# arkworks-rs/groth16

Hardware: AMD Instinct MI355X
Metric: R1CS constraints/sec (create_proof, BLS12-381) (higher is better)
Workload: dtype u32-limb Montgomery integers (Fr 255-bit, Fq 381-bit); 1 GPU; SYN(k=22) synthetic R1CS, 4194302 constraints, FFT domain 2^22, bls12_381, full create_proof (7 NTTs + 4 G1 MSMs + 1 G2 MSM), valid proving key generated on the GPU from seeded toxic waste; curve=bls12_381, log2_domain=22, constraints=4194302, key=valid, witness=resident in HBM at entry (--full: value_incl_h2d holds the PCIe-inclusive rates), parallelism=single-gpu

## Files before the change

### groth16_amd/csrc/msm.hip

```cpp
#include "internal.hpp"
#include "msm_common.hpp"
#include "fp30.hpp"
#include "batch_affine.hpp"
#include "window_tables.hpp"
#include <algorithm>
#include <cstdlib>

namespace g16 {

static constexpr int SORT_THREADS = 1024;
static constexpr int ACC_THREADS = 64;
static constexpr int RED_THREADS = 64;
static constexpr int WIN_THREADS = 256;
#ifndef G16_REDUCE_G
#define G16_REDUCE_G 8
#endif
static constexpr uint32_t REDUCE_G = G16_REDUCE_G;

struct PlanDev {
    int c, W;
    uint32_t B;
    uint32_t K[10];
    uint32_t shard_n, shard_r, shard_magic;
};
// ... 81 lines not shown
    __syncthreads();
    const uint64_t i = (uint64_t)blockIdx.x * CLASS_THREADS + threadIdx.x;
    if (i < n) {
        biased_scalar(scalars[i], plan, sw);
        for (int w = 0; w < plan.W; ++w) {
            uint32_t key, neg;
            if (digit_to_bucket(window_of(sw, w, plan.c), plan.c, &key, &neg) && shard_local_key(plan, &key)) atomicAdd(&cnt[key >> blog], 1u);
        }
    }
    __syncthreads();
    if (threadIdx.x < Q) block_counts[(uint64_t)threadIdx.x * gridDim.x + blockIdx.x] = cnt[threadIdx.x];
}

template <class Fr>
__global__ __launch_bounds__(CLASS_THREADS) void class_partition_kernel(const Fr* __restrict__ scalars, uint64_t n, PlanDev plan, uint32_t blog,
                                                                        uint32_t Q, const uint32_t* __restrict__ block_off,
                                                                        uint16_t* __restrict__ ent_key, uint32_t* __restrict__ ent_tag) {
    __shared__ uint32_t sw[MSM_SWORDS][CLASS_THREADS];
    __shared__ uint32_t cur[MAX_CLASSES];
    if (threadIdx.x < Q) cur[threadIdx.x] = block_off[(uint64_t)threadIdx.x * gridDim.x + blockIdx.x];
    __syncthreads();
    const uint64_t i = (uint64_t)blockIdx.x * CLASS_THREADS + threadIdx.x;
    if (i >= n) return;
    biased_scalar(scalars[i], plan, sw);
    for (int w = 0; w < plan.W; ++w) {
        uint32_t key, neg;
        if (digit_to_bucket(window_of(sw, w, plan.c), plan.c, &key, &neg) && shard_local_key(plan, &key)) {
            const uint32_t pos = atomicAdd(&cur[key >> blog], 1u);
            ent_key[pos] = (uint16_t)((key & ((1u << blog) - 1u)) | (neg << 15));
            ent_tag[pos] = (uint32_t)i | ((uint32_t)w << 26);
        }
    }
}

static __global__ __launch_bounds__(SORT_M_THREADS) void bucket_count_merged_kernel(const uint16_t* __restrict__ ent_key,
                                                                           const uint32_t* __restrict__ class_off, uint32_t nb, uint32_t B,
                                                                           uint32_t* __restrict__ wg_counts) {
    extern __shared__ __attribute__((aligned(16))) unsigned char smem[];
    uint32_t* hist = reinterpret_cast<uint32_t*>(smem);
    const uint32_t q = blockIdx.y;
    const uint32_t lo = class_off[(uint64_t)q * nb], hi = class_off[(uint64_t)(q + 1) * nb];
    for (uint32_t b = threadIdx.x; b < B; b += SORT_M_THREADS) hist[b] = 0;
    __syncthreads();
    for (uint64_t p = (uint64_t)lo + blockIdx.x * SORT_M_THREADS + threadIdx.x; p < hi; p += (uint64_t)gridDim.x * SORT_M_THREADS)
        atomicAdd(&hist[ent_key[p] & 0x7fffu], 1u);
    __syncthreads();
    uint32_t* out = wg_counts + ((uint64_t)q * gridDim.x + blockIdx.x) * B;
    for (uint32_t b = threadIdx.x; b < B; b += SORT_M_THREADS) out[b] = hist[b];
}

static __global__ __launch_bounds__(256) void bucket_wg_scan_kernel(uint32_t* __restrict__ wg_counts, uint32_t G, uint32_t B, uint32_t M,
                                                                    uint32_t* __restrict__ counts) {
    const uint32_t i = blockIdx.x * 256 + threadIdx.x;
    if (i >= M) return;
    const uint32_t q = i / B, b = i - q * B;
    uint32_t* col = wg_counts + (uint64_t)q * G * B + b;
    uint32_t run = 0;
    for (uint32_t x = 0; x < G; ++x) {
        const uint32_t v = col[(uint64_t)x * B];
        col[(uint64_t)x * B] = run;
        run += v;
    }
    counts[i] = run;
}

static __global__ __launch_bounds__(SORT_M_THREADS) void bucket_scatter_merged_kernel(const uint16_t* __restrict__ ent_key,
                                                                             const uint32_t* __restrict__ ent_tag,
                                                                             const uint32_t* __restrict__ class_off, uint32_t nb, uint32_t B,
                                                                             const uint32_t* __restrict__ offsets,
                                                                             const uint32_t* __restrict__ wg_counts, uint32_t* __restrict__ sorted) {
    extern __shared__ __attribute__((aligned(16))) unsigned char smem[];
    uint32_t* hist = reinterpret_cast<uint32_t*>(smem);
    const uint32_t q = blockIdx.y;
    const uint32_t lo = class_off[(uint64_t)q * nb], hi = class_off[(uint64_t)(q + 1) * nb];
    if ((uint64_t)lo + (uint64_t)blockIdx.x * SORT_M_THREADS >= hi) return;
    const uint64_t qb = (uint64_t)q * B;
    const uint32_t* mine = wg_counts + ((uint64_t)q * gridDim.x + blockIdx.x) * B;
    for (uint32_t b = threadIdx.x; b < B; b += SORT_M_THREADS) hist[b] = offsets[qb + b] + mine[b];
    __syncthreads();
    const uint64_t first = (uint64_t)lo + blockIdx.x * SORT_M_THREADS + threadIdx.x, step = (uint64_t)gridDim.x * SORT_M_THREADS;
    for (uint64_t p = first; p < hi; p += step) {
        const uint32_t d = ent_key[p];
        const uint32_t pos = atomicAdd(&hist[d & 0x7fffu], 1u);
        sorted[pos] = ent_tag[p] | ((d >> 15) << 31);
    }
}

static constexpr int SCAN_THREADS = 256;
static constexpr int SCAN_PER_THREAD = 8;
static constexpr int SCAN_TILE = SCAN_THREADS * SCAN_PER_THREAD;
static constexpr uint32_t HEAVY_PARTS = 16;

__device__ __forceinline__ uint32_t block_exclusive(uint32_t v, uint32_t* sh, uint32_t* total) {
    const uint32_t tid = threadIdx.x;
    sh[tid] = v;
    __syncthreads();
    for (uint32_t d = 1; d < SCAN_THREADS; d <<= 1) {
        const uint32_t add = tid >= d ? sh[tid - d] : 0u;
        __syncthreads();
        sh[tid] += add;
        __syncthreads();
    }
    const uint32_t incl = sh[tid];
    *total = sh[SCAN_THREADS - 1];
    __syncthreads();
    return incl - v;
}

static __global__ __launch_bounds__(SCAN_THREADS) void scan_block_sums_kernel(const uint32_t* __restrict__ vals, uint32_t M, uint32_t pad,
                                                                       uint32_t* __restrict__ block_sums) {
    __shared__ uint32_t sa[SCAN_THREADS];
    const uint32_t base = blockIdx.x * SCAN_TILE + threadIdx.x * SCAN_PER_THREAD;
    uint32_t sum = 0, tot;
    G16_UNROLL for (int j = 0; j < SCAN_PER_THREAD; ++j) sum += (base + j < M) ? ((vals[base + j] + pad) & ~pad) : 0u;
    (void)block_exclusive(sum, sa, &tot);
    if (threadIdx.x == 0) block_sums[blockIdx.x] = tot;
}

static __global__ __launch_bounds__(SCAN_THREADS) void scan_block_offsets_kernel(uint32_t* __restrict__ block_sums, uint32_t nblocks, uint32_t M,
                                                                          uint32_t* __restrict__ prefix) {
    __shared__ uint32_t sa[SCAN_THREADS];
    uint32_t carry = 0;
    for (uint32_t base = 0; base < nblocks; base += SCAN_THREADS) {
        const uint32_t i = base + threadIdx.x;
        const uint32_t a = i < nblocks ? block_sums[i] : 0u;
        uint32_t tot;
        const uint32_t ea = block_exclusive(a, sa, &tot);
        if (i < nblocks) block_sums[i] = carry + ea;
        carry += tot;
    }
    if (threadIdx.x == 0) prefix[M] = carry;
}

static __global__ __launch_bounds__(SCAN_THREADS) void scan_write_kernel(const uint32_t* __restrict__ vals, uint32_t M, uint32_t pad,
                                                                  const uint32_t* __restrict__ block_base, uint32_t* __restrict__ prefix) {
    __shared__ uint32_t sa[SCAN_THREADS];
    const uint32_t base = blockIdx.x * SCAN_TILE + threadIdx.x * SCAN_PER_THREAD;
    uint32_t cv[SCAN_PER_THREAD], sum = 0, tot;
    G16_UNROLL for (int j = 0; j < SCAN_PER_THREAD; ++j) { cv[j] = (base + j < M) ? ((vals[base + j] + pad) & ~pad) : 0u; sum += cv[j]; }
    uint32_t a = block_base[blockIdx.x] + block_exclusive(sum, sa, &tot);
    G16_UNROLL for (int j = 0; j < SCAN_PER_THREAD; ++j) {
        if (base + j < M) { prefix[base + j] = a; a += cv[j]; }
    }
}

static __global__ void bucket_slots_kernel(const uint32_t* __restrict__ offsets, uint32_t M, uint32_t off_shift, uint32_t lseg,
                                    uint32_t* __restrict__ nparts, uint32_t* __restrict__ heavy ) {
    const uint32_t b = blockIdx.x * blockDim.x + threadIdx.x;
    if (b >= M) return;
    const uint32_t lo = offsets[b] >> off_shift, hi = offsets[b + 1] >> off_shift;
    const uint32_t np = hi > lo ? ((hi - 1) / lseg - lo / lseg + 1u) : 0u;
    nparts[b] = np;
    if (np > HEAVY_PARTS) heavy[1 + atomicAdd(&heavy[0], 1u)] = b;
}

static __global__ __launch_bounds__(SORT_THREADS) void bucket_scatter_kernel(const uint16_t* __restrict__ planes, uint64_t n, uint32_t chunk,
                                                                      int c, uint32_t B, const uint32_t* __restrict__ offsets,
                                                                      uint32_t* __restrict__ cursor, uint32_t* __restrict__ sorted) {
    extern __shared__ __attribute__((aligned(16))) unsigned char smem[];
    uint32_t* hist = reinterpret_cast<uint32_t*>(smem);
    const int w = blockIdx.y;
    for (uint32_t b = threadIdx.x; b < B; b += SORT_THREADS) hist[b] = 0;
    __syncthreads();
    const uint64_t lo = (uint64_t)blockIdx.x * chunk, hi = min(n, lo + chunk);
    const uint16_t* plane = planes + (uint64_t)w * n;
    for (uint64_t p = lo + threadIdx.x; p < hi; p += SORT_THREADS) {
        uint32_t bucket, neg;
        if (digit_to_bucket(plane[p], c, &bucket, &neg)) atomicAdd(&hist[bucket], 1u);
    }
    __syncthreads();
    const uint64_t wb = (uint64_t)w * B;
    for (uint32_t b = threadIdx.x; b < B; b += SORT_THREADS) {
        const uint32_t v = hist[b];
        if (v) hist[b] = offsets[wb + b] + atomicAdd(&cursor[wb + b], v);
    }
    __syncthreads();
    for (uint64_t p = lo + threadIdx.x; p < hi; p += SORT_THREADS) {
        uint32_t bucket, neg;
        if (digit_to_bucket(plane[p], c, &bucket, &neg)) {
            const uint32_t pos = atomicAdd(&hist[bucket], 1u);
            sorted[pos] = (uint32_t)p | (neg << 31);
        }
    }
}

template <class F30>
struct LdsAccStore {
    static constexpr int NL = F30::PREFIX_LIMBS;
    static constexpr int QUADS = NL / 4, TAIL = NL % 4;
    static constexpr int WORDS_PER_VALUE = NL * ACC_THREADS;
    uint32_t* quad;
    uint32_t* tail;
    __device__ __forceinline__ F30 ld(int v) const {
        asm volatile("" ::: "memory");
        uint32_t w[NL];
        const uint32_t* q = quad + v * WORDS_PER_VALUE;
        G16_UNROLL for (int g = 0; g < QUADS; ++g) {
            const uint4 t = *reinterpret_cast<const uint4*>(q + g * 4 * ACC_THREADS);
            w[4 * g] = t.x; w[4 * g + 1] = t.y; w[4 * g + 2] = t.z; w[4 * g + 3] = t.w;
        }
        const uint32_t* r = tail + v * WORDS_PER_VALUE;
        G16_UNROLL for (int i = 0; i < TAIL; ++i) w[4 * QUADS + i] = r[i * ACC_THREADS];
        return F30::from_limbs(w);
    }
    __device__ __forceinline__ void st(int v, const F30& a) const {
        uint32_t w[NL];
        a.get_limbs(w);
        uint32_t* q = quad + v * WORDS_PER_VALUE;
        G16_UNROLL for (int g = 0; g < QUADS; ++g)
            *reinterpret_cast<uint4*>(q + g * 4 * ACC_THREADS) = make_uint4(w[4 * g], w[4 * g + 1], w[4 * g + 2], w[4 * g + 3]);
        uint32_t* r = tail + v * WORDS_PER_VALUE;
        G16_UNROLL for (int i = 0; i < TAIL; ++i) r[i * ACC_THREADS] = w[4 * QUADS + i];
        asm volatile("" ::: "memory");
    }
};

template <class F30>
struct RawAccStore {
    AccRaw<typename F30::Raw>* p;
    __device__ __forceinline__ F30 ld(int k) const {
        asm volatile("" ::: "memory");
        if constexpr (F30::LANES_PER_TASK == 1) {
            static_assert(sizeof(F30) == sizeof(typename F30::Raw), "one-lane fields share the raw layout");
            return reinterpret_cast<const F30*>(p)[k];
        } else {
            typedef typename F30::B B30;
            return F30{reinterpret_cast<const B30*>(p)[2 * k + (F30::lane_hi() ? 1 : 0)]};
        }
    }
    __device__ __forceinline__ void st(int k, const F30& a) const {
        if constexpr (F30::LANES_PER_TASK == 1) {
            reinterpret_cast<F30*>(p)[k] = a;
        } else {
            typedef typename F30::B B30;
            reinterpret_cast<B30*>(p)[2 * k + (F30::lane_hi() ? 1 : 0)] = a.c;
        }
        asm volatile("" ::: "memory");
    }
    __device__ __forceinline__ bool inf() const {
        const F30 zz = ld(2);
        if constexpr (F30::LANES_PER_TASK == 1) return zz.raw_zero();
        else return F30::both(zz.c.raw_zero());
    }
    __device__ __forceinline__ void set_inf() const { st(2, F30::zero()); }
};
template <class F30>
struct RegAccStore {
    F30 v[4];
    __device__ __forceinline__ F30 ld(int k) const { return v[k]; }
    __device__ __forceinline__ void st(int k, const F30& a) { v[k] = a; }
};
template <class F30, class St>
__device__ __forceinline__ Acc30<F30> gather_acc(const St& st, bool inf) {
    Acc30<F30> a;
    a.inf = inf;
    if (inf) { a.x = a.y = a.zz = a.zzz = F30::zero(); return a; }
    a.x = st.ld(0); a.y = st.ld(1); a.zz = st.ld(2); a.zzz = st.ld(3);
    return a;
}

static constexpr int PASS_BATCH = 4;
template <class F30>
struct PassBatch {
    const Affine<typename F30::Std>* bases[PASS_BATCH];
    int64_t shift[PASS_BATCH];
    uint64_t base_count[PASS_BATCH];
    const uint32_t* sorted[PASS_BATCH];
    const uint32_t* offsets[PASS_BATCH];
    const uint32_t* slot_off[PASS_BATCH];
    AccRaw<typename F30::Raw>* partials[PASS_BATCH];
};

template <class F30, bool DIRECT>
__global__ __launch_bounds__(ACC_THREADS, F30::ACC_MIN_WAVES) void bucket_accumulate30_kernel(
    PassBatch<F30> batch, uint32_t M, uint32_t off_shift, uint32_t lseg, uint32_t merged) {
    const Affine<typename F30::Std>* __restrict__ bases = batch.bases[blockIdx.y];
    const int64_t shift = batch.shift[blockIdx.y];
    const uint64_t base_count = batch.base_count[blockIdx.y];
    const uint32_t* __restrict__ sorted = batch.sorted[blockIdx.y];
    const uint32_t* __restrict__ offsets = batch.offsets[blockIdx.y];
    const uint32_t* __restrict__ slot_off = batch.slot_off[blockIdx.y];
    AccRaw<typename F30::Raw>* __restrict__ partials = batch.partials[blockIdx.y];
    const uint32_t t = (blockIdx.x * ACC_THREADS + threadIdx.x) / F30::LANES_PER_TASK;
    const uint32_t S = offsets[M] >> off_shift;
    const uint64_t start64 = (uint64_t)t * lseg;
    if (start64 >= S) return;
    const uint32_t start = (uint32_t)start64;
    const uint32_t end = (uint32_t)min((uint64_t)S, start64 + lseg);
    uint32_t lo = 0, hi = M;
    while (hi - lo > 1) {
        const uint32_t mid = (lo + hi) >> 1;
        if ((offsets[mid] >> off_shift) <= start) lo = mid; else hi = mid;
    }
    uint32_t b = lo, b_first = offsets[b] >> off_shift, b_end = offsets[b + 1] >> off_shift;
    __shared__ __attribute__((aligned(16))) uint32_t acc_lds[4 * F30::PREFIX_LIMBS * ACC_THREADS];
    AccParked<F30, LdsAccStore<F30>> acc;
    acc.s.quad = acc_lds + 4 * threadIdx.x;
    acc.s.tail = acc_lds + 4 * LdsAccStore<F30>::QUADS * ACC_THREADS + threadIdx.x;
    acc.inf = true;
    auto flush = [&](AccRaw<typename F30::Raw>* dst) { acc.gather().store_raw(dst); acc.inf = true; };
    uint32_t v_next = 0;
    typedef typename F30::PackedC YNext;
    F30 px_next = F30::zero();
    YNext py_next = YNext::zero();
    bool ok_next = false;
    auto decode = [&](uint32_t v, int64_t* at) -> bool {
// ... 266 lines not shown
}

int make_msm_plan(uint64_t n, int scalar_bits, const uint32_t* modulus_words, int mod_nwords, int merged_c, MsmPlan* plan, int shard_n,
                  int shard_r) {
    if (shard_n < 1 || shard_n > 64 || shard_r < 0 || shard_r >= shard_n || (shard_n > 1 && merged_c <= 0)) return G16_ERR_INTERNAL;
    int c = merged_c;
    if (c <= 0) {
        c = msm_window_override();
        if (c <= 0) {
            double best = 1e300;
            for (int cc = 4; cc <= 16; ++cc) {
                const int W = plan_windows(cc, scalar_bits, modulus_words, mod_nwords, nullptr);
                if (W < 0) continue;
                const double t = plan_cost(n, W, (double)W * (1u << (cc - 1)), W);
                if (t < best) { best = t; c = cc; }
            }
        }
        if (c < 3) c = 3;
        if (c > 16) c = 16;
    } else if (c < MSM_MERGED_MIN_C || c > MSM_MERGED_MAX_C || n > MSM_MERGED_MAX_N) {
        return G16_ERR_INTERNAL;
    }
    const int W = plan_windows(c, scalar_bits, modulus_words, mod_nwords, plan->K);
    if (W < 0 || (merged_c > 0 && W > 32)) return G16_ERR_INTERNAL;
    plan->c = c;
    plan->W = W;
    plan->merged = merged_c > 0;
    plan->shard_n = shard_n;
    plan->shard_r = shard_r;
    if (plan->merged) {
        const uint32_t all = 1u << (c - 1), local = (all + (uint32_t)shard_n - 1) / (uint32_t)shard_n;
        uint32_t B = 1;
        while (B < local && B < (1u << 15)) B <<= 1;
        plan->B = B;
        plan->groups = (int)((local + B - 1) / B);
    } else {
        plan->B = 1u << (c - 1);
        plan->groups = W;
    }
    plan->G = REDUCE_G;
    if (const char* e = getenv("G16_MSM_REDUCE_G")) {
        const int v = atoi(e);
        if (v == 4 || v == 8 || v == 16 || v == 32) plan->G = (uint32_t)v;
    }
    const uint64_t all_entries = n * (uint64_t)W / (uint64_t)shard_n;
    plan->affine_levels = 0;
    {
        const uint64_t mean_load = all_entries / plan->buckets();
        (void)mean_load;
        int R = 0;
        if (const char* e = getenv("G16_MSM_AFFINE_LEVELS")) {
            const int v = atoi(e);
            if (v >= 0 && v <= 4) R = v;
        }
        if (all_entries + (uint64_t)plan->buckets() * ((1u << R) - 1u) >= ((uint64_t)1 << 32)) R = 0;
        if (shard_n > 1) R = 0;
        plan->affine_levels = R;
    }
    const uint64_t entries = (all_entries >> plan->affine_levels) + (plan->affine_levels ? plan->buckets() : 0);
    uint32_t l = 64;
    while (l > 16 && entries / l < 4ull * 131072ull) l >>= 1;
    const uint64_t mean = entries / plan->buckets() + 1;
    while (l < 128 && (uint64_t)l * 4 < mean) l <<= 1;
    if (const char* e = getenv("G16_MSM_SEGMENT")) {
        const int v = atoi(e);
        if (v >= 8 && v <= 4096) l = (uint32_t)v;
    }
    plan->Lmax = l;
    uint64_t nchunks = 2048 / (uint64_t)plan->groups;
    if (nchunks < 1) nchunks = 1;
    uint64_t chunk = (n + nchunks - 1) / nchunks;
    chunk = (chunk + 1023) / 1024 * 1024;
    if (chunk < 1024) chunk = 1024;
    plan->chunk = (uint32_t)chunk;
    return G16_OK;
}

#endif

static int ilog2(uint32_t v) { int l = 0; while ((1u << l) < v) ++l; return l; }

template <class C>
int sort_scalars(const typename C::Fr* d_scalars, uint64_t n, int merged_c, Arena& arena, hipStream_t st, ScalarSort* out, int shard_n,
                 int shard_r) {
    typedef typename C::Fr Fr;
    if (n >= ((uint64_t)1 << 31)) return G16_ERR_BAD_LENGTH;
    uint32_t modw[Fr::N];
    for (int i = 0; i < Fr::N; ++i) modw[i] = Fr::Params::mod(i);
    MsmPlan plan;
    G16_TRY(make_msm_plan(n, Fr::Params::BITS, modw, Fr::N, merged_c, &plan, shard_n, shard_r));
    out->plan = plan;
    out->n = n;
    const uint32_t M = plan.buckets();
    const uint64_t nw = n * (uint64_t)plan.W;
    if (nw >= ((uint64_t)1 << 32)) return G16_ERR_BAD_LENGTH;
    uint16_t* planes = nullptr;
    uint32_t* ent_tag = nullptr;
    uint32_t *class_cnt = nullptr, *class_off = nullptr;
    uint32_t *counts = nullptr, *cursor = nullptr, *nparts = nullptr, *block_sums = nullptr;
    uint32_t sort_class_log = SORT_CLASS_LOG;
    if (const char* e = getenv("G16_SORT_CLASS_LOG")) {
        const int v = atoi(e);
        if (v >= 8 && v <= 15) sort_class_log = (uint32_t)v;
    }
    const uint32_t slog = plan.merged ? std::min<uint32_t>(sort_class_log, (uint32_t)ilog2(plan.B)) : 0u;
    const uint32_t Bs = plan.merged ? 1u << slog : plan.B;
    const uint32_t nb = (uint32_t)((n + CLASS_THREADS - 1) / CLASS_THREADS), Q = plan.merged ? M >> slog : (uint32_t)plan.groups;
    G16_TRY(arena.alloc_n(nw ? nw : 1, &planes));
    if (plan.merged) {
        if (Q > MAX_CLASSES) return G16_ERR_INTERNAL;
        G16_TRY(arena.alloc_n(nw ? nw : 1, &ent_tag));
        G16_TRY(arena.alloc_n((size_t)Q * nb + 1, &class_cnt));
        G16_TRY(arena.alloc_n((size_t)Q * nb + 1, &class_off));
    }
    G16_TRY(arena.alloc_n((size_t)3 * M + 1, &counts));
    cursor = counts + M;
    out->heavy = counts + 2 * (size_t)M;
    G16_TRY(arena.alloc_n((size_t)M + 1, &out->offsets));
    G16_TRY(arena.alloc_n((size_t)M + 1, &out->task_off));
    G16_TRY(arena.alloc_n((size_t)M, &nparts));
    const int R = plan.affine_levels;
    const uint32_t pad = (1u << R) - 1u;
    const uint64_t max_sorted = nw + (uint64_t)M * pad;
    if (max_sorted >= ((uint64_t)1 << 32)) return G16_ERR_BAD_LENGTH;
    out->max_sorted = max_sorted;
    G16_TRY(arena.alloc_n(max_sorted ? max_sorted : 1, &out->sorted));
    if (R) G16_HIP_TRY(hipMemsetAsync(out->sorted, 0xff, max_sorted * sizeof(uint32_t), st));
    const uint64_t walked = R ? (max_sorted >> R) : nw;
    out->max_segments = (uint32_t)((walked + plan.Lmax - 1) / plan.Lmax);
    out->max_tasks = out->max_segments + M;
    G16_HIP_TRY(hipMemsetAsync(counts, 0, ((size_t)2 * M + 1) * sizeof(uint32_t), st));
    PlanDev pd;
    pd.c = plan.c; pd.W = plan.W; pd.B = plan.B;
    for (int k = 0; k < 10; ++k) pd.K[k] = plan.K[k];
    pd.shard_n = (uint32_t)plan.shard_n;
    pd.shard_r = (uint32_t)plan.shard_r;
    pd.shard_magic = plan.shard_n > 1 ? (uint32_t)((((uint64_t)1 << 32) + (uint64_t)plan.shard_n - 1) / (uint64_t)plan.shard_n) : 0u;
    const size_t lds = (size_t)Bs * sizeof(uint32_t);
    static PerDeviceOnce attr_once;
    std::atomic<bool>& attr_set = attr_once.flag();
    if (!attr_set) {
        G16_HIP_TRY(hipFuncSetAttribute(reinterpret_cast<const void*>(&bucket_count_kernel), hipFuncAttributeMaxDynamicSharedMemorySize,
                                        128 * 1024));
        G16_HIP_TRY(hipFuncSetAttribute(reinterpret_cast<const void*>(&bucket_scatter_kernel), hipFuncAttributeMaxDynamicSharedMemorySize,
                                        128 * 1024));
        G16_HIP_TRY(hipFuncSetAttribute(reinterpret_cast<const void*>(&bucket_count_merged_kernel),
                                        hipFuncAttributeMaxDynamicSharedMemorySize, 128 * 1024));
        G16_HIP_TRY(hipFuncSetAttribute(reinterpret_cast<const void*>(&bucket_scatter_merged_kernel),
                                        hipFuncAttributeMaxDynamicSharedMemorySize, 128 * 1024));
        attr_set = true;
    }
    const unsigned nchunks = (unsigned)((n + plan.chunk - 1) / plan.chunk);
    const uint32_t blog = plan.merged ? slog : (uint32_t)ilog2(plan.B);
    const uint32_t max_scan = std::max(M, plan.merged ? Q * nb : 0u);
    G16_TRY(arena.alloc_n((size_t)(max_scan + SCAN_TILE - 1) / SCAN_TILE, &block_sums));
    auto prefix_scan = [&](const uint32_t* vals, uint32_t* prefix, uint32_t count, uint32_t padmask = 0) -> int {
        const uint32_t nblocks = (count + SCAN_TILE - 1) / SCAN_TILE;
        hipLaunchKernelGGL(scan_block_sums_kernel, dim3(nblocks), dim3(SCAN_THREADS), 0, st, vals, count, padmask, block_sums);
        G16_LAUNCH_CHECK();
        hipLaunchKernelGGL(scan_block_offsets_kernel, dim3(1), dim3(SCAN_THREADS), 0, st, block_sums, nblocks, count, prefix);
        G16_LAUNCH_CHECK();
        hipLaunchKernelGGL(scan_write_kernel, dim3(nblocks), dim3(SCAN_THREADS), 0, st, vals, count, padmask, block_sums, prefix);
        G16_LAUNCH_CHECK();
        return G16_OK;
    };
    unsigned gx = std::max(1u, std::min(std::min(4096u / Q, 256u), (unsigned)((nw + SORT_M_THREADS - 1) / SORT_M_THREADS)));
    if (const char* e = getenv("G16_SORT_GX")) {
        const int v = atoi(e);
        if (v >= 1 && v <= 4096) gx = (unsigned)v;
    }
    uint32_t* wg_counts = nullptr;
    if (plan.merged) G16_TRY(arena.alloc_n((size_t)Q * gx * Bs, &wg_counts));
    if (n) {
        if (plan.merged) {
            hipLaunchKernelGGL((class_count_kernel<Fr>), dim3(nb), dim3(CLASS_THREADS), 0, st, d_scalars, n, pd, blog, Q, class_cnt);
            G16_LAUNCH_CHECK();
            G16_TRY(prefix_scan(class_cnt, class_off, Q * nb));
            hipLaunchKernelGGL((class_partition_kernel<Fr>), dim3(nb), dim3(CLASS_THREADS), 0, st, d_scalars, n, pd, blog, Q, class_off, planes,
                               ent_tag);
            G16_LAUNCH_CHECK();
            hipLaunchKernelGGL(bucket_count_merged_kernel, dim3(gx, Q), dim3(SORT_M_THREADS), lds, st, planes, class_off, nb, Bs, wg_counts);
            G16_LAUNCH_CHECK();
            hipLaunchKernelGGL(bucket_wg_scan_kernel, dim3((M + 255) / 256), dim3(256), 0, st, wg_counts, gx, Bs, M, counts);
        } else {
            hipLaunchKernelGGL((digits_kernel<Fr>), dim3((unsigned)((n + 255) / 256)), dim3(256), 0, st, d_scalars, n, pd, planes);
            G16_LAUNCH_CHECK();
            hipLaunchKernelGGL(bucket_count_kernel, dim3(nchunks, plan.W), dim3(SORT_THREADS), lds, st, planes, n, plan.chunk, plan.c, plan.B,
                               counts);
        }
        G16_LAUNCH_CHECK();
    }
    G16_TRY(prefix_scan(counts, out->offsets, M, pad));
    hipLaunchKernelGGL(bucket_slots_kernel, dim3((M + 255) / 256), dim3(256), 0, st, out->offsets, M, (uint32_t)R, plan.Lmax, nparts,
                       out->heavy);
    G16_LAUNCH_CHECK();
    G16_TRY(prefix_scan(nparts, out->task_off, M));
    if (n) {
        if (plan.merged)
            hipLaunchKernelGGL(bucket_scatter_merged_kernel, dim3(gx, Q), dim3(SORT_M_THREADS), lds, st, planes, ent_tag, class_off, nb, Bs,
                               out->offsets, wg_counts, out->sorted);
        else
            hipLaunchKernelGGL(bucket_scatter_kernel, dim3(nchunks, plan.W), dim3(SORT_THREADS), lds, st, planes, n, plan.chunk, plan.c, plan.B,
                               out->offsets, cursor, out->sorted);
        G16_LAUNCH_CHECK();
    }
    return G16_OK;
}

template <class F>
static int alloc_msm_buffers(const ScalarSort& ss, Arena& arena, MsmBuffers<F>* out) {
    typedef AccRaw<typename Lazy30<F>::type::Raw> Raw;
    const MsmPlan& plan = ss.plan;
    const uint32_t cpw = plan.B / plan.chunk_buckets();
    Raw *partials = nullptr, *chunk_out = nullptr;
    G16_TRY(arena.alloc_n((size_t)ss.max_tasks ? ss.max_tasks : 1, &partials));
    G16_TRY(arena.alloc_n((size_t)cpw * plan.groups * 2, &chunk_out));
    G16_TRY(arena.alloc_n((size_t)plan.outputs(), &out->window_sums));
    out->partials = partials;
    out->chunk_out = chunk_out;
    return G16_OK;
}

template <class F>
int msm_bucket_pass(const Affine<F>* d_bases, int64_t shift, uint64_t base_count, const ScalarSort& ss, Arena& arena, hipStream_t st,
                    MsmBuffers<F>* out, EventTimer* bucket_timer) {
    typedef typename Lazy30<F>::type F30;
    typedef AccRaw<typename Lazy30<F>::type::Raw> Raw;
    const MsmPlan& plan = ss.plan;
    const uint32_t M = plan.buckets();
    const int R = plan.affine_levels;
    if (!R || !ss.max_sorted) {
        const PassJob<F> job{d_bases, shift, base_count, &ss, out};
        return msm_bucket_pass_batch<F>(&job, 1, arena, st, bucket_timer);
    }
    G16_TRY(alloc_msm_buffers<F>(ss, arena, out));
    Raw* partials = static_cast<Raw*>(out->partials);
    Affine<F>* lists[2] = {nullptr, nullptr};
    Word4* prefix = nullptr;
    constexpr uint32_t T = 64 / F30::LANES_PER_TASK;
    constexpr int QUADS = AffineLevel<F30, true>::QUADS;
    auto level_K = [&](int r) -> uint32_t {
        const uint64_t pairs = ss.max_sorted >> (r + 1);
        uint32_t K = 64;
        while (K > 8 && pairs / ((uint64_t)K * T) < 2048) K >>= 1;
        return K;
    };
    auto level_waves = [&](int r) -> uint64_t { return ((ss.max_sorted >> (r + 1)) + (uint64_t)level_K(r) * T - 1) / ((uint64_t)level_K(r) * T); };
    {
        G16_TRY(arena.alloc_n((size_t)(ss.max_sorted >> 1) + 1, &lists[0]));
        if (R > 1) G16_TRY(arena.alloc_n((size_t)(ss.max_sorted >> 2) + 1, &lists[1]));
        size_t recs = 0;
        for (int r = 0; r < R; ++r) recs = std::max(recs, (size_t)(level_waves(r) * level_K(r)) * QUADS * 64);
        G16_TRY(arena.alloc_n(recs ? recs : 1, &prefix));
    }
    if (bucket_timer) G16_TRY(bucket_timer->start(st));
    {
        AffineLevelArgs<F30> a;
        a.sorted = ss.sorted;
        a.total = ss.offsets + M;
        a.prefix = prefix;
        a.shift = shift;
        a.base_count = base_count;
        a.merged = plan.merged ? 1u : 0u;
        for (int r = 0; r < R; ++r) {
            a.in = r == 0 ? d_bases : lists[(r - 1) & 1];
            a.out = lists[r & 1];
            a.level = (uint32_t)r;
            a.K = level_K(r);
            const uint64_t waves = level_waves(r);
            const unsigned blocks = (unsigned)((waves * 64 + AFF_THREADS - 1) / AFF_THREADS);
            if (r == 0) hipLaunchKernelGGL((affine_level_kernel<F30, true>), dim3(blocks), dim3(AFF_THREADS), 0, st, a);
            else hipLaunchKernelGGL((affine_level_kernel<F30, false>), dim3(blocks), dim3(AFF_THREADS), 0, st, a);
            G16_LAUNCH_CHECK();
        }
    }
    if (ss.max_segments) {
        const uint64_t lanes = (uint64_t)ss.max_segments * F30::LANES_PER_TASK;
        const dim3 grid((unsigned)((lanes + ACC_THREADS - 1) / ACC_THREADS));
        PassBatch<F30> b;
        for (int i = 0; i < PASS_BATCH; ++i) {
            b.bases[i] = lists[(R - 1) & 1]; b.shift[i] = 0; b.base_count[i] = 0; b.sorted[i] = nullptr;
            b.offsets[i] = ss.offsets; b.slot_off[i] = ss.task_off; b.partials[i] = partials;
        }
        hipLaunchKernelGGL((bucket_accumulate30_kernel<F30, true>), grid, dim3(ACC_THREADS), 0, st, b, M, (uint32_t)R, plan.Lmax, 0u);
        G16_LAUNCH_CHECK();
    }
    if (bucket_timer) G16_TRY(bucket_timer->stop(st));
    return G16_OK;
}

template <class F30>
static unsigned pass_lds_pad() {
    static const int want = [] { const char* e = getenv("G16_PASS_WG_PER_CU"); return e ? atoi(e) : 0; }();
    if (want <= 0) return 0;
    const unsigned own = 4u * F30::PREFIX_LIMBS * ACC_THREADS * 4u;
    const unsigned per = (160u * 1024u / (unsigned)want) & ~255u;
    return per > own ? per - own : 0;
}

template <class F>
int msm_bucket_pass_batch(const PassJob<F>* jobs, int n, Arena& arena, hipStream_t st, EventTimer* bucket_timer) {
    typedef typename Lazy30<F>::type F30;
    typedef AccRaw<typename Lazy30<F>::type::Raw> Raw;
    if (n < 1 || n > PASS_BATCH) return G16_ERR_INTERNAL;
    const MsmPlan& plan = jobs[0].ss->plan;
    for (int i = 0; i < n; ++i) {
        const MsmPlan& q = jobs[i].ss->plan;
        if (q.B != plan.B || q.groups != plan.groups || q.Lmax != plan.Lmax || q.merged != plan.merged) return G16_ERR_INTERNAL;
        if (q.affine_levels && jobs[i].ss->max_sorted) return G16_ERR_INTERNAL;
    }
    PassBatch<F30> b;
    uint32_t max_segments = 0;
    for (int i = 0; i < n; ++i) G16_TRY(alloc_msm_buffers<F>(*jobs[i].ss, arena, jobs[i].out));
    for (int i = 0; i < PASS_BATCH; ++i) {
        const PassJob<F>& j = jobs[i < n ? i : 0];
        b.bases[i] = j.bases; b.shift[i] = j.shift; b.base_count[i] = j.base_count; b.sorted[i] = j.ss->sorted;
        b.offsets[i] = j.ss->offsets; b.slot_off[i] = j.ss->task_off; b.partials[i] = static_cast<Raw*>(j.out->partials);
        if (i < n) max_segments = std::max(max_segments, j.ss->max_segments);
    }
    if (bucket_timer) G16_TRY(bucket_timer->start(st));
    if (max_segments) {
        const uint64_t lanes = (uint64_t)max_segments * F30::LANES_PER_TASK;
        const dim3 grid((unsigned)((lanes + ACC_THREADS - 1) / ACC_THREADS), (unsigned)n);
        hipLaunchKernelGGL((bucket_accumulate30_kernel<F30, false>), grid, dim3(ACC_THREADS), pass_lds_pad<F30>(), st, b, plan.buckets(), 0u,
                           plan.Lmax, plan.merged ? 1u : 0u);
        G16_LAUNCH_CHECK();
    }
    if (bucket_timer) G16_TRY(bucket_timer->stop(st));
    return G16_OK;
}

template <class F>
static int reduce_setup(size_t* lds_heavy, size_t* lds_win) {
    typedef typename Lazy30<F>::type F30;
    typedef AccRaw<typename F30::Raw> Raw;
    static PerDeviceOnce attr_once;
    std::atomic<bool>& attr_set = attr_once.flag();
    *lds_heavy = sizeof(Raw) * HEAVY_THREADS / F30::LANES_PER_TASK;
    *lds_win = sizeof(Raw) * WIN_THREADS / F30::LANES_PER_TASK;
    if (!attr_set) {
        G16_HIP_TRY(hipFuncSetAttribute(reinterpret_cast<const void*>(&heavy_reduce_kernel<F30>), hipFuncAttributeMaxDynamicSharedMemorySize,
                                        (int)*lds_heavy));
        G16_HIP_TRY(hipFuncSetAttribute(reinterpret_cast<const void*>(&window_reduce_kernel<F30>), hipFuncAttributeMaxDynamicSharedMemorySize,
                                        (int)*lds_win));
        attr_set = true;
    }
    return G16_OK;
}

template <class F>
// ... 189 lines not shown
```

Before: 68.09 million constraints/s.

## Replace merged bucket count/scatter with two-level LDS radix sort for MSM buckets

For the merged-plan, unsharded case, the per-workgroup bucket histogram plus global-atomic scatter is replaced by a two-level sort. The first level partitions entries by high key bits into sub-ranges, using per-tile LDS staging so global writes are coalesced. The second level sorts each sub-range in LDS and writes bucket counts and sorted words. This targets scattered global writes and the large wg_counts scan, at the cost of an extra pass over keys and tags, extra buffers, and LDS-capacity assumptions (FINAL_CAP) that fall back to direct global writes when exceeded.

```diff
diff --git a/groth16_amd/csrc/msm.hip b/groth16_amd/csrc/msm.hip
--- a/groth16_amd/csrc/msm.hip
+++ b/groth16_amd/csrc/msm.hip
@@ -257,6 +257,158 @@
     const uint32_t np = hi > lo ? ((hi - 1) / lseg - lo / lseg + 1u) : 0u;
     nparts[b] = np;
     if (np > HEAVY_PARTS) heavy[1 + atomicAdd(&heavy[0], 1u)] = b;
+}
+
+static constexpr uint32_t MAX_SUBS = 256;
+static constexpr uint32_t MAX_SUB_LOG = 7;
+static constexpr uint32_t SUB_TILE = 4096;
+static constexpr uint32_t SUB_PER_LANE = SUB_TILE / SORT_M_THREADS;
+static constexpr uint32_t SUB_BATCH = 4;
+static constexpr uint32_t FINAL_CAP = 10240;
+static constexpr uint32_t FINAL_BATCH = 4;
+static_assert(SORT_M_THREADS == SCAN_THREADS && MAX_SUBS <= SCAN_THREADS && SUB_TILE <= 65536, "block_exclusive scans one value per lane");
+
+__device__ __forceinline__ uint32_t lds_take(uint32_t* ctr, uint32_t idx, bool valid) {
+    const uint64_t act = __ballot(valid);
+    if (act == 0) return 0;
+    const int first = __ffsll((unsigned long long)act) - 1;
+    const uint32_t idx0 = (uint32_t)__shfl((int)idx, first);
+    if (__ballot(valid && idx == idx0) == act) {
+        const uint32_t lane = threadIdx.x & 63u;
+        uint32_t base = 0;
+        if ((int)lane == first) base = atomicAdd(&ctr[idx0], (uint32_t)__popcll(act));
+        base = (uint32_t)__shfl((int)base, first);
+        return base + (uint32_t)__popcll(act & (((uint64_t)1 << lane) - 1u));
+    }
+    return valid ? atomicAdd(&ctr[idx], 1u) : 0u;
+}
+
+static __global__ __launch_bounds__(SORT_M_THREADS) void sub_count_kernel(const uint16_t* __restrict__ ent_key,
+                                                                          const uint32_t* __restrict__ class_off, uint32_t nb, uint32_t S,
+                                                                          uint32_t sublog, uint32_t* __restrict__ sub_counts) {
+    __shared__ uint32_t cnt[MAX_SUBS];
+    const uint32_t q = blockIdx.y;
+    const uint64_t lo = class_off[(uint64_t)q * nb], hi = class_off[(uint64_t)(q + 1) * nb];
+    cnt[threadIdx.x] = 0;
+    __syncthreads();
+    for (uint64_t tlo = lo + (uint64_t)blockIdx.x * SUB_TILE; tlo < hi; tlo += (uint64_t)gridDim.x * SUB_TILE) {
+        uint32_t k[SUB_PER_LANE];
+        G16_UNROLL for (uint32_t j = 0; j < SUB_PER_LANE; ++j) {
+            const uint64_t p = tlo + j * SORT_M_THREADS + threadIdx.x;
+            k[j] = p < hi ? (uint32_t)ent_key[p] : 0xffffffffu;
+        }
+        G16_UNROLL for (uint32_t j = 0; j < SUB_PER_LANE; ++j) (void)lds_take(cnt, (k[j] & 0x7fffu) >> sublog, k[j] != 0xffffffffu);
+    }
+    __syncthreads();
+    if (threadIdx.x < S) sub_counts[((uint64_t)q * S + threadIdx.x) * gridDim.x + blockIdx.x] = cnt[threadIdx.x];
+}
+
+static __global__ __launch_bounds__(SORT_M_THREADS) void sub_partition_kernel(const uint16_t* __restrict__ ent_key,
+                                                                              const uint32_t* __restrict__ ent_tag,
+                                                                              const uint32_t* __restrict__ class_off, uint32_t nb, uint32_t S,
+                                                                              uint32_t sublog, const uint32_t* __restrict__ sub_off,
+                                                                              uint16_t* __restrict__ out_key, uint32_t* __restrict__ out_tag) {
+    __shared__ uint32_t cnt[MAX_SUBS], start[MAX_SUBS], cur[MAX_SUBS], gcur[MAX_SUBS], sa[SCAN_THREADS];
+    __shared__ uint32_t stag[SUB_TILE];
+    __shared__ uint16_t skey[SUB_TILE];
+    const uint32_t q = blockIdx.y;
+    const uint64_t lo = class_off[(uint64_t)q * nb], hi = class_off[(uint64_t)(q + 1) * nb];
+    if (lo + (uint64_t)blockIdx.x * SUB_TILE >= hi) return;
+    gcur[threadIdx.x] = threadIdx.x < S ? sub_off[((uint64_t)q * S + threadIdx.x) * gridDim.x + blockIdx.x] : 0u;
+    cnt[threadIdx.x] = 0;
+    __syncthreads();
+    for (uint64_t tlo = lo + (uint64_t)blockIdx.x * SUB_TILE; tlo < hi; tlo += (uint64_t)gridDim.x * SUB_TILE) {
+        const uint32_t tn = (uint32_t)min((uint64_t)SUB_TILE, hi - tlo);
+        _Pragma("unroll 1") for (uint32_t i0 = 0; i0 < tn; i0 += SUB_BATCH * SORT_M_THREADS) {
+            uint32_t k[SUB_BATCH];
+            G16_UNROLL for (uint32_t j = 0; j < SUB_BATCH; ++j) {
+                const uint32_t i = i0 + j * SORT_M_THREADS + threadIdx.x;
+                k[j] = i < tn ? (uint32_t)ent_key[tlo + i] : 0xffffffffu;
+            }
+            G16_UNROLL for (uint32_t j = 0; j < SUB_BATCH; ++j) (void)lds_take(cnt, (k[j] & 0x7fffu) >> sublog, k[j] != 0xffffffffu);
+        }
+        __syncthreads();
+        uint32_t tot;
+        const uint32_t mine = cnt[threadIdx.x], ex = block_exclusive(mine, sa, &tot);
+        start[threadIdx.x] = ex;
+        cur[threadIdx.x] = ex;
+        __syncthreads();
+        _Pragma("unroll 1") for (uint32_t i0 = 0; i0 < tn; i0 += SUB_BATCH * SORT_M_THREADS) {
+            uint32_t k[SUB_BATCH], t[SUB_BATCH];
+            G16_UNROLL for (uint32_t j = 0; j < SUB_BATCH; ++j) {
+                const uint32_t i = i0 + j * SORT_M_THREADS + threadIdx.x;
+                k[j] = i < tn ? (uint32_t)ent_key[tlo + i] : 0xffffffffu;
+                t[j] = i < tn ? ent_tag[tlo + i] : 0u;
+            }
+            G16_UNROLL for (uint32_t j = 0; j < SUB_BATCH; ++j) {
+                const bool valid = k[j] != 0xffffffffu;
+                const uint32_t pos = lds_take(cur, (k[j] & 0x7fffu) >> sublog, valid);
+                if (valid) {
+                    skey[pos] = (uint16_t)k[j];
+                    stag[pos] = t[j];
+                }
+            }
+        }
+        __syncthreads();
+        _Pragma("unroll 1") for (uint32_t i = threadIdx.x; i < tn; i += SORT_M_THREADS) {
+            const uint32_t key = skey[i], s = (key & 0x7fffu) >> sublog;
+            const uint32_t g = gcur[s] + (i - start[s]);
+            out_key[g] = (uint16_t)key;
+            out_tag[g] = stag[i];
+        }
+        __syncthreads();
+        gcur[threadIdx.x] += mine;
+        cnt[threadIdx.x] = 0;
+        __syncthreads();
+    }
+}
+
+static __global__ __launch_bounds__(SORT_M_THREADS) void final_sort_kernel(const uint16_t* __restrict__ ent_key,
+                                                                           const uint32_t* __restrict__ ent_tag,
+                                                                           const uint32_t* __restrict__ sub_off, uint32_t G, uint32_t sublog,
+                                                                           uint32_t* __restrict__ counts, uint32_t* __restrict__ sorted) {
+    __shared__ uint32_t cnt[1u << MAX_SUB_LOG], cur[1u << MAX_SUB_LOG], sa[SCAN_THREADS];
+    __shared__ uint32_t out[FINAL_CAP];
+    const uint32_t u = blockIdx.x, NB = 1u << sublog;
+    const uint64_t lo = sub_off[(uint64_t)u * G], hi = sub_off[(uint64_t)(u + 1) * G];
+    if (threadIdx.x < NB) cnt[threadIdx.x] = 0;
+    __syncthreads();
+    for (uint64_t base = lo; base < hi; base += 2 * FINAL_BATCH * SORT_M_THREADS) {
+        uint32_t k[2 * FINAL_BATCH];
+        G16_UNROLL for (uint32_t j = 0; j < 2 * FINAL_BATCH; ++j) {
+            const uint64_t p = base + j * SORT_M_THREADS + threadIdx.x;
+            k[j] = p < hi ? (uint32_t)ent_key[p] : 0xffffffffu;
+        }
+        G16_UNROLL for (uint32_t j = 0; j < 2 * FINAL_BATCH; ++j) (void)lds_take(cnt, k[j] & (NB - 1u), k[j] != 0xffffffffu);
+    }
+    __syncthreads();
+    const uint32_t mine = threadIdx.x < NB ? cnt[threadIdx.x] : 0u;
+    if (threadIdx.x < NB) counts[((uint64_t)u << sublog) + threadIdx.x] = mine;
+    uint32_t tot;
+    const uint32_t ex = block_exclusive(mine, sa, &tot);
+    if (threadIdx.x < NB) cur[threadIdx.x] = ex;
+    __syncthreads();
+    const bool resident = hi - lo <= FINAL_CAP;
+    for (uint64_t base = lo; base < hi; base += FINAL_BATCH * SORT_M_THREADS) {
+        uint32_t k[FINAL_BATCH], t[FINAL_BATCH];
+        G16_UNROLL for (uint32_t j = 0; j < FINAL_BATCH; ++j) {
+            const uint64_t p = base + j * SORT_M_THREADS + threadIdx.x;
+            k[j] = p < hi ? (uint32_t)ent_key[p] : 0xffffffffu;
+            t[j] = p < hi ? ent_tag[p] : 0u;
+        }
+        G16_UNROLL for (uint32_t j = 0; j < FINAL_BATCH; ++j) {
+            const bool valid = k[j] != 0xffffffffu;
+            const uint32_t pos = lds_take(cur, k[j] & (NB - 1u), valid), word = t[j] | ((k[j] >> 15) << 31);
+            if (valid) {
+                if (resident) out[pos] = word;
+                else sorted[lo + pos] = word;
+            }
+        }
+    }
+    if (!resident) return;
+    __syncthreads();
+    const uint32_t N = (uint32_t)(hi - lo);
+    for (uint32_t i = threadIdx.x; i < N; i += SORT_M_THREADS) sorted[lo + i] = out[i];
 }
 
 static __global__ __launch_bounds__(SORT_THREADS) void bucket_scatter_kernel(const uint16_t* __restrict__ planes, uint64_t n, uint32_t chunk,
@@ -829,7 +981,20 @@
     }
     const unsigned nchunks = (unsigned)((n + plan.chunk - 1) / plan.chunk);
     const uint32_t blog = plan.merged ? slog : (uint32_t)ilog2(plan.B);
-    const uint32_t max_scan = std::max(M, plan.merged ? Q * nb : 0u);
+    const bool two_level = plan.merged && R == 0;
+    uint32_t sublog = 0, S = 1;
+    unsigned gx2 = 1;
+    if (two_level) {
+        const uint64_t mean_x4 = 4 * (nw / (uint64_t)plan.shard_n) / M + 1;
+        const uint32_t lo_log = slog > 8 ? slog - 8 : 0u;
+        sublog = std::min<uint32_t>(slog, MAX_SUB_LOG);
+        while (sublog > lo_log && (mean_x4 << sublog) > 3 * (uint64_t)FINAL_CAP) --sublog;
+        if (sublog > MAX_SUB_LOG) return G16_ERR_INTERNAL;
+        S = Bs >> sublog;
+        gx2 = std::max(1u, std::min(std::min(4096u / Q, 256u), (unsigned)((nw + SUB_TILE - 1) / SUB_TILE)));
+    }
+    const uint32_t sub_cells = two_level ? Q * S * gx2 : 0u;
+    const uint32_t max_scan = std::max(std::max(M, plan.merged ? Q * nb : 0u), sub_cells);
     G16_TRY(arena.alloc_n((size_t)(max_scan + SCAN_TILE - 1) / SCAN_TILE, &block_sums));
     auto prefix_scan = [&](const uint32_t* vals, uint32_t* prefix, uint32_t count, uint32_t padmask = 0) -> int {
         const uint32_t nblocks = (count + SCAN_TILE - 1) / SCAN_TILE;
@@ -847,7 +1012,15 @@
         if (v >= 1 && v <= 4096) gx = (unsigned)v;
     }
     uint32_t* wg_counts = nullptr;
-    if (plan.merged) G16_TRY(arena.alloc_n((size_t)Q * gx * Bs, &wg_counts));
+    if (plan.merged && !two_level) G16_TRY(arena.alloc_n((size_t)Q * gx * Bs, &wg_counts));
+    uint16_t* sub_key = nullptr;
+    uint32_t *sub_tag = nullptr, *sub_cnt = nullptr, *sub_off = nullptr;
+    if (two_level) {
+        G16_TRY(arena.alloc_n(nw ? nw : 1, &sub_key));
+        G16_TRY(arena.alloc_n(nw ? nw : 1, &sub_tag));
+        G16_TRY(arena.alloc_n((size_t)sub_cells + 1, &sub_cnt));
+        G16_TRY(arena.alloc_n((size_t)sub_cells + 1, &sub_off));
+    }
     if (n) {
         if (plan.merged) {
             hipLaunchKernelGGL((class_count_kernel<Fr>), dim3(nb), dim3(CLASS_THREADS), 0, st, d_scalars, n, pd, blog, Q, class_cnt);
@@ -856,9 +1029,21 @@
             hipLaunchKernelGGL((class_partition_kernel<Fr>), dim3(nb), dim3(CLASS_THREADS), 0, st, d_scalars, n, pd, blog, Q, class_off, planes,
                                ent_tag);
             G16_LAUNCH_CHECK();
-            hipLaunchKernelGGL(bucket_count_merged_kernel, dim3(gx, Q), dim3(SORT_M_THREADS), lds, st, planes, class_off, nb, Bs, wg_counts);
-            G16_LAUNCH_CHECK();
-            hipLaunchKernelGGL(bucket_wg_scan_kernel, dim3((M + 255) / 256), dim3(256), 0, st, wg_counts, gx, Bs, M, counts);
+            if (two_level) {
+                hipLaunchKernelGGL(sub_count_kernel, dim3(gx2, Q), dim3(SORT_M_THREADS), 0, st, planes, class_off, nb, S, sublog, sub_cnt);
+                G16_LAUNCH_CHECK();
+                G16_TRY(prefix_scan(sub_cnt, sub_off, sub_cells));
+                hipLaunchKernelGGL(sub_partition_kernel, dim3(gx2, Q), dim3(SORT_M_THREADS), 0, st, planes, ent_tag, class_off, nb, S, sublog,
+                                   sub_off, sub_key, sub_tag);
+                G16_LAUNCH_CHECK();
+                hipLaunchKernelGGL(final_sort_kernel, dim3(Q * S), dim3(SORT_M_THREADS), 0, st, sub_key, sub_tag, sub_off, gx2, sublog, counts,
+                                   out->sorted);
+            } else {
+                hipLaunchKernelGGL(bucket_count_merged_kernel, dim3(gx, Q), dim3(SORT_M_THREADS), lds, st, planes, class_off, nb, Bs,
+                                   wg_counts);
+                G16_LAUNCH_CHECK();
+                hipLaunchKernelGGL(bucket_wg_scan_kernel, dim3((M + 255) / 256), dim3(256), 0, st, wg_counts, gx, Bs, M, counts);
+            }
         } else {
             hipLaunchKernelGGL((digits_kernel<Fr>), dim3((unsigned)((n + 255) / 256)), dim3(256), 0, st, d_scalars, n, pd, planes);
             G16_LAUNCH_CHECK();
@@ -872,7 +1057,7 @@
                        out->heavy);
     G16_LAUNCH_CHECK();
     G16_TRY(prefix_scan(nparts, out->task_off, M));
-    if (n) {
+    if (n && !two_level) {
         if (plan.merged)
             hipLaunchKernelGGL(bucket_scatter_merged_kernel, dim3(gx, Q), dim3(SORT_M_THREADS), lds, st, planes, ent_tag, class_off, nb, Bs,
                                out->offsets, wg_counts, out->sorted);
```

After: 69.87 million constraints/s (median of 6 runs). +2.6%, better.
